# shicaiwei123/ICCV2025-GDL

Measured on AMD Instinct MI355X. Metric: audio-visual samples/sec, CREMA-D DGL train step (whole job), higher is better.
Workload: dtype bf16; 1 GPU; CREMA-D DGL (main_dgl.py, ConcatFusion_DGL) ResNet18 a+v, spec 1x257x188 + frames 3x3x224x224, alpha=4, SGD lr 2e-3 mom .9 wd 1e-4, clip 40; per_gpu_batch=64, global_batch=64, parallelism=dp1, buckets=none

## Files before the change

### iccv2025-gdl_amd/csrc/conv_wgrad.hip

```cpp
#include <stdlib.h>

#include "common.h"
#include "gather.h"
#include "prof.h"

#include <hip/hip_ext.h>

namespace gdl {

struct WgradArgs {
    const void* dy;
    const void* x;
    float* partial;
    const GatherEntry* table;
    int C, K, RS, M;
    int nsplit, chunk;
    int tiles_k, tiles_c;
    unsigned dy_bytes, x_bytes;
    int delta[9];
    int split;
    int delta_hi[9];
#ifdef GDL_TIMING
    unsigned long long* dbg;
#endif
};
#ifdef GDL_TIMING
extern unsigned long long* g_timing_buf;
#endif

constexpr int WG_BP = 64;

__device__ __forceinline__ uint2 lds_tr16(const unsigned char* p) {
    s16x4_t v = __builtin_amdgcn_ds_read_tr16_b64_v4i16((__attribute__((address_space(3))) s16x4_t*)(p));
    return __builtin_bit_cast(uint2, v);
}

__device__ __forceinline__ void wg_dma16(__amdgpu_buffer_rsrc_t rsrc, unsigned char* lds_base, int voffset) {
#if defined(__HIP_DEVICE_COMPILE__)
    __builtin_amdgcn_raw_ptr_buffer_load_lds(rsrc, (__attribute__((address_space(3))) void*)lds_base, 16, voffset, 0, 0, 0);
#else
    (void)rsrc;
    (void)lds_base;
    (void)voffset;
#endif
}
__device__ __forceinline__ uint2 lds_tr16_asm(unsigned addr) {
    uint2 v;
    asm volatile("ds_read_b64_tr_b16 %0, %1" : "=v"(v) : "v"(addr));
    return v;
}
__device__ __forceinline__ float lds_read_f32_asm(unsigned addr) {
    float v;
    asm volatile("ds_read_b32 %0, %1" : "=v"(v) : "v"(addr));
    return v;
}
__device__ __forceinline__ void wg_lds_wait() {
    asm volatile("s_waitcnt lgkmcnt(0)" ::: "memory");
    __builtin_amdgcn_sched_barrier(0);
}

template <int PITCH>
__device__ __forceinline__ int wg_swz(int row) {
    if (PITCH == 128) return ((row >> 1) & 1) | (((row >> 3) & 1) << 1);
    return (row & 3) | (((row >> 3) & 1) << 2);
}

template <typename T, int TK, int TC>
__global__ __launch_bounds__(256) void conv_wgrad_kernel(WgradArgs a) {
    extern __shared__ __attribute__((aligned(16))) unsigned char smem[];
    constexpr int PK = TK * (int)sizeof(T), PC = TC * (int)sizeof(T);
    constexpr int STAGE = WG_BP * (PK + PC);
    constexpr int CPR_K = PK / 16, CPR_C = PC / 16;
    constexpr int LK = WG_BP * CPR_K / 256, LC = WG_BP * CPR_C / 256;
    constexpr int WTK = TK / 2, WTC = TC / 2, FK = WTK / 16, FC = WTC / 16;

    const int tid = threadIdx.x, lane = tid & 63, wave = tid >> 6;
    const int wk = wave & 1, wc = wave >> 1;

    const int RS = a.RS;
    const int per_slice = RS * a.tiles_k * a.tiles_c;
    const int L = xcd_linear(a.nsplit * per_slice);
    if (L < 0) return;
    const int slice = L / per_slice;
    int rem = L - slice * per_slice;
    const int tap = rem % RS;
    rem /= RS;
    const int kt = rem % a.tiles_k, ct = rem / a.tiles_k;
    const int k0 = kt * TK, c0 = ct * TC;

    const int m_begin = slice * a.chunk;
    const int m_end = min(a.M, m_begin + a.chunk);
    const int nst = (m_end - m_begin + WG_BP - 1) / WG_BP;

    const __amdgpu_buffer_rsrc_t rdy = __builtin_amdgcn_make_buffer_rsrc((void*)a.dy, 0, a.dy_bytes, 0x00020000);
    const __amdgpu_buffer_rsrc_t rx = __builtin_amdgcn_make_buffer_rsrc((void*)a.x, 0, a.x_bytes, 0x00020000);
    const int esz = (int)sizeof(T);
    const int tap_delta = a.delta[tap] + c0 * esz;
    int dy_off[LK];
#pragma unroll
    for (int i = 0; i < LK; ++i) {
        const int idx = tid + 256 * i;
        const int row = idx / CPR_K, pc = idx % CPR_K;
        const int ch = (((pc >> 1) ^ wg_swz<PK>(row)) << 1) | (pc & 1);
        dy_off[i] = (m_begin + row) * (a.K * esz) + k0 * esz + ch * 16;
    }
    int x_ch[LC];
    bool x_hi[LC];
#pragma unroll
    for (int i = 0; i < LC; ++i) {
        const int idx = tid + 256 * i;
        const int row = idx / CPR_C, pc = idx % CPR_C;
        const int lc = (((pc >> 1) ^ wg_swz<PC>(row)) << 1) | (pc & 1);
        x_hi[i] = a.split && lc >= CPR_C / 2;
        x_ch[i] = (x_hi[i] ? lc - CPR_C / 2 : lc) * 16;
    }
    const int tap_delta_hi = a.delta_hi[tap];
    GatherEntry ent[LC];
#pragma unroll
    for (int i = 0; i < LC; ++i) {
        const int idx = tid + 256 * i;
        const int m = m_begin + idx / CPR_C;
        ent[i].off0 = 0;
        ent[i].mask = 0;
        if (m < m_end) ent[i] = a.table[m];
    }
    int ld_m = m_begin;
    const int wbase = (tid >> 6) * 64 * 16;

    auto load_stage = [&](int buf) {
        unsigned char* Ks = smem + buf * STAGE;
        unsigned char* Cs = Ks + WG_BP * PK;
#pragma unroll
        for (int i = 0; i < LK; ++i) {
            const int idx = tid + 256 * i;
            const int m = ld_m + idx / CPR_K;
            wg_dma16(rdy, Ks + 256 * 16 * i + wbase, m < m_end ? dy_off[i] : (int)0x80000000);
            dy_off[i] += WG_BP * a.K * esz;
        }
#pragma unroll
        for (int i = 0; i < LC; ++i) {
            const int v = ((ent[i].mask >> tap) & 1u) ? ent[i].off0 + (x_hi[i] ? tap_delta_hi : tap_delta) + x_ch[i]
                                                      : (int)0x80000000;
            wg_dma16(rx, Cs + 256 * 16 * i + wbase, v);
        }
        ld_m += WG_BP;
#pragma unroll
        for (int i = 0; i < LC; ++i) {
            const int idx = tid + 256 * i;
            const int m = ld_m + idx / CPR_C;
            GatherEntry e;
            e.off0 = 0;
            e.mask = 0;
            if (m < m_end) e = a.table[m];
            ent[i] = e;
        }
    };

    f32x4_t acc[FK][FC];
#pragma unroll
    for (int i = 0; i < FK; ++i)
#pragma unroll
        for (int jj = 0; jj < FC; ++jj) acc[i][jj] = f32x4_t{0.f, 0.f, 0.f, 0.f};

    const int g = lane >> 4, li = lane & 15;

    const unsigned smem_base = (unsigned)(uintptr_t)(const __attribute__((address_space(3))) unsigned char*)smem;
#ifdef GDL_TIMING
    unsigned long long t_entry = __builtin_amdgcn_s_memtime(), t_wait = 0, t_comp = 0, t_issue = 0, t_a, t_b;
#endif
    if (nst > 0) load_stage(0);
#ifdef GDL_TIMING
    unsigned long long t_first = __builtin_amdgcn_s_memtime();
#endif
    for (int st = 0; st < nst; ++st) {
        const int buf = st & 1;
#ifdef GDL_TIMING
        t_a = __builtin_amdgcn_s_memtime();
#endif
        asm volatile("s_waitcnt vmcnt(0)" ::: "memory");
        __builtin_amdgcn_s_barrier();
        asm volatile("" ::: "memory");
#ifdef GDL_TIMING
        t_b = __builtin_amdgcn_s_memtime();
        t_wait += t_b - t_a;
#endif
        if (st + 1 < nst) load_stage(buf ^ 1);
#ifdef GDL_TIMING
        t_a = __builtin_amdgcn_s_memtime();
        t_issue += t_a - t_b;
#endif
        const unsigned Ks = smem_base + buf * STAGE;
        const unsigned Cs = Ks + WG_BP * PK;
        if (sizeof(T) == 2) {
#pragma unroll
            for (int ks = 0; ks < WG_BP / 32; ++ks) {
                uint2 alo[FK], ahi[FK], blo[FC], bhi[FC];
#pragma unroll
                for (int h = 0; h < 2; ++h) {
                    const int row = ks * 32 + g * 8 + h * 4 + (li >> 2);
#pragma unroll
                    for (int i = 0; i < FK; ++i) {
                        const int chb = (wk * WTK + i * 16 + (li & 3) * 4) * 2;
                        const int addr = row * PK + ((((chb >> 5) ^ wg_swz<PK>(row)) << 5) | (chb & 31));
                        if (h == 0)
                            alo[i] = lds_tr16_asm(Ks + addr);
                        else
                            ahi[i] = lds_tr16_asm(Ks + addr);
                    }
#pragma unroll
                    for (int jj = 0; jj < FC; ++jj) {
                        const int chb = (wc * WTC + jj * 16 + (li & 3) * 4) * 2;
                        const int addr = row * PC + ((((chb >> 5) ^ wg_swz<PC>(row)) << 5) | (chb & 31));
                        if (h == 0)
                            blo[jj] = lds_tr16_asm(Cs + addr);
                        else
                            bhi[jj] = lds_tr16_asm(Cs + addr);
                    }
                }
                wg_lds_wait();
#pragma unroll
                for (int i = 0; i < FK; ++i) {
                    const uint4 fa = make_uint4(alo[i].x, alo[i].y, ahi[i].x, ahi[i].y);
#pragma unroll
                    for (int jj = 0; jj < FC; ++jj) {
                        const uint4 fb = make_uint4(blo[jj].x, blo[jj].y, bhi[jj].x, bhi[jj].y);
                        acc[i][jj] = __builtin_amdgcn_mfma_f32_16x16x32_bf16(__builtin_bit_cast(bf16x8_t, fa),
                                                                           __builtin_bit_cast(bf16x8_t, fb), acc[i][jj], 0,
                                                                           0, 0);
                    }
                }
            }
        } else {
#pragma unroll 4
            for (int ks = 0; ks < WG_BP / 4; ++ks) {
                const int row = ks * 4 + g;
                float fa[FK], fb[FC];
#pragma unroll
                for (int i = 0; i < FK; ++i) {
                    const int chb = (wk * WTK + i * 16 + li) * 4;
                    fa[i] = lds_read_f32_asm(Ks + row * PK + ((((chb >> 5) ^ wg_swz<PK>(row)) << 5) | (chb & 31)));
                }
#pragma unroll
                for (int jj = 0; jj < FC; ++jj) {
                    const int chb = (wc * WTC + jj * 16 + li) * 4;
                    fb[jj] = lds_read_f32_asm(Cs + row * PC + ((((chb >> 5) ^ wg_swz<PC>(row)) << 5) | (chb & 31)));
                }
                wg_lds_wait();
#pragma unroll
                for (int i = 0; i < FK; ++i)
#pragma unroll
                    for (int jj = 0; jj < FC; ++jj)
                        acc[i][jj] = __builtin_amdgcn_mfma_f32_16x16x4f32(fa[i], fb[jj], acc[i][jj], 0, 0, 0);
            }
        }
    }
#ifdef GDL_TIMING
    unsigned long long t_loop_end = __builtin_amdgcn_s_memtime();
    t_comp = (t_loop_end - t_first) - t_wait - t_issue;
#endif
    float* part = a.partial + (size_t)slice * a.K * RS * a.C;
#pragma unroll
    for (int i = 0; i < FK; ++i)
#pragma unroll
        for (int jj = 0; jj < FC; ++jj) {
            const int c = c0 + wc * WTC + jj * 16 + li;
#pragma unroll
            for (int e = 0; e < 4; ++e) {
                const int k = k0 + wk * WTK + i * 16 + g * 4 + e;
                part[((size_t)k * RS + tap) * a.C + c] = acc[i][jj][e];
            }
        }
#ifdef GDL_TIMING
    if (a.dbg && tid == 0) {
        unsigned long long* d = a.dbg + (size_t)blockIdx.x * 8;
        d[0] = t_entry;
        d[1] = t_first - t_entry;
        d[2] = t_wait;
        d[3] = t_issue;
        d[4] = t_comp;
        d[5] = __builtin_amdgcn_s_memtime() - t_loop_end;
        d[6] = nst;
    }
#endif
}

template <int LANES>
__global__ __launch_bounds__(256) void wgrad_reduce_kernel(const float* __restrict__ partial, float* __restrict__ out,
                                                           int nsplit, int K, int RS, int C, int Cout) {
    constexpr int OUTS = 256 / LANES;
    __shared__ float red[LANES][OUTS];
    const size_t total = (size_t)K * RS * C;
    const int o = threadIdx.x % OUTS, l = threadIdx.x / OUTS;
    const size_t i = blockIdx.x * (size_t)OUTS + o;
    float s = 0.f;
    if (i < total)
        for (int sp = l; sp < nsplit; sp += LANES) s += partial[(size_t)sp * total + i];
    if (LANES > 1) {
        red[l][o] = s;
        __syncthreads();
        if (l == 0) {
            s = red[0][o];
#pragma unroll
            for (int j = 1; j < LANES; ++j) s += red[j][o];
        }
    }
    if (l == 0 && i < total) {
        const int c = (int)(i % C);
        const size_t t = i / C;
        const int rs = (int)(t % RS);
        const int k = (int)(t / RS);
        if (c < Cout) out[((size_t)k * Cout + c) * RS + rs] = s;
    }
}

bool conv_wgrad9_enabled();
bool conv_wgrad9_ok(int dtype, int W, int C, int K, int R, int S, int stride, int pad);
size_t conv_wgrad9_ws_bytes(int M, int C, int K);
int conv_wgrad9(const void* dy, const void* x, float* dw, const void* table, int N, int H, int W, int C, int K, void* ws,
                size_t ws_bytes, hipStream_t st);

struct WgradPlan {
    int tk, tc, nsplit, chunk;
};

static WgradPlan plan_wgrad(int M, int C, int K, int RS, bool gemm = false) {
    WgradPlan p;
    p.tk = (K % 128 == 0) ? 128 : 64;
    p.tc = (C % 128 == 0) ? 128 : 64;
    const int tiles = (K / p.tk) * (C / p.tc) * RS;
    static int forced = -1;
    if (forced < 0) {
        const char* e = tune_env("GDL_WGRAD_BLOCKS");
        forced = e ? atoi(e) : 0;
    }
    static int forced_gemm = -1;
    if (forced_gemm < 0) {
        const char* e = tune_env("GDL_WGRAD_GEMM_BLOCKS");
        forced_gemm = e ? atoi(e) : 0;
    }
    const int target = (gemm && forced_gemm > 0) ? forced_gemm : forced > 0 ? forced : (gemm ? 416 : 128);
    int ns = (target + tiles - 1) / tiles;
    const int max_ns = (M + 2 * WG_BP - 1) / (2 * WG_BP);
    if (ns > max_ns) ns = max_ns;
    if (ns < 1) ns = 1;
    int chunk = (M + ns - 1) / ns;
    chunk = (chunk + WG_BP - 1) / WG_BP * WG_BP;
    p.nsplit = (M + chunk - 1) / chunk;
    p.chunk = chunk;
    return p;
}

size_t conv_wgrad_ws_bytes(int M, int C, int K, int RS) {
    const WgradPlan p = plan_wgrad(M, C, K, RS, RS == 1);
    size_t b = (size_t)p.nsplit * K * RS * C * sizeof(float);
    if (RS == 9 && conv_wgrad9_enabled()) {
        const size_t b9 = conv_wgrad9_ws_bytes(M, C, K);
        if (b9 > b) b = b9;
    }
    return b;
}

template <typename T, int TK, int TC>
static int launch_wg(WgradArgs& a, hipStream_t st) {
    constexpr int BYTES = 2 * WG_BP * (TK + TC) * (int)sizeof(T);
    auto kfn = conv_wgrad_kernel<T, TK, TC>;
    static DevOnce attr_set;
    if (!attr_set) {
        hipError_t e = hipFuncSetAttribute((const void*)kfn, hipFuncAttributeMaxDynamicSharedMemorySize, BYTES);
        if (e != hipSuccess) return check_hip(e, "hipFuncSetAttribute(conv_wgrad)");
        attr_set = true;
    }
    const int per_slice = a.RS * a.tiles_k * a.tiles_c;
    const int grid = xcd_grid(a.nsplit * per_slice);
    static char pname[96] = "";
    if (!pname[0]) snprintf(pname, sizeof(pname), "gdl::conv_wgrad_kernel<%s, %d, %d>", prof_tname<T>(), TK, TC);
    ProfScope prof(pname, PROF_MFMA, st, 2.0 * (double)a.M * a.K * a.C * a.RS, true,
                   (double)a.dy_bytes + (double)a.x_bytes + 4.0 * (double)a.K * a.C * a.RS);
    hipExtLaunchKernelGGL(kfn, dim3(grid), dim3(256), BYTES, st, prof.e0(), prof.e1(), 0, a);
    GDL_CHECK_LAUNCH("conv_wgrad_kernel");
    return GDL_OK;
}

int conv_wgrad(int dtype, const void* dy, const void* x, float* dw, const void* table, int N, int H, int W, int C, int K,
               int R, int S, int stride, int pad, int Cout, void* ws, size_t ws_bytes, hipStream_t st) {
    GDL_REQUIRE(dtype == GDL_BF16 || dtype == GDL_F32, "wgrad: bad dtype %d", dtype);
    GDL_REQUIRE(table, "wgrad: gather table is null (build it with gdl_conv_build_table)");
    GDL_REQUIRE(C % 64 == 0 && K % 64 == 0, "wgrad: C=%d K=%d must be multiples of 64", C, K);
    if (Cout == C && conv_wgrad9_ok(dtype, W, C, K, R, S, stride, pad))
        return conv_wgrad9(dy, x, dw, table, N, H, W, C, K, ws, ws_bytes, st);
    GatherGeom g;
    int rc = gather_geom(GATHER_FWD, dtype, N, H, W, C, K, R, S, stride, pad, &g);
    if (rc) return rc;
    const int esz = dtype == GDL_BF16 ? 2 : 4;
    WgradArgs a{};
#ifdef GDL_TIMING
    a.dbg = g_timing_buf;
#endif
    a.dy = dy;
    a.x = x;
    a.table = (const GatherEntry*)table;
    a.C = C;
    a.K = K;
    a.RS = R * S;
    a.M = g.rows;
    for (int t = 0; t < 9; ++t) a.delta[t] = g.delta[t];
    GDL_REQUIRE(a.M < (1 << 24), "wgrad: M exceeds 2^24");
    GDL_REQUIRE((size_t)a.M * K * esz < (1UL << 31), "wgrad: dy exceeds 2 GiB");
    a.dy_bytes = (unsigned)((size_t)a.M * K * esz);
    a.x_bytes = (unsigned)((size_t)N * H * W * C * esz);
    const WgradPlan p = plan_wgrad(a.M, C, K, R * S, R == 1 && S == 1 && stride == 1);
    a.nsplit = p.nsplit;
    a.chunk = p.chunk;
    a.tiles_k = K / p.tk;
    a.tiles_c = C / p.tc;
    const size_t need = (size_t)p.nsplit * K * R * S * C * sizeof(float);
    if (ws_bytes < need || !ws) {
        set_error("wgrad: workspace %zu < %zu bytes", ws_bytes, need);
        return GDL_ERR_WORKSPACE;
    }
    a.partial = (float*)ws;
    if (dtype == GDL_BF16) {
        if (p.tk == 128 && p.tc == 128)
            rc = launch_wg<bf16, 128, 128>(a, st);
        else if (p.tk == 128)
            rc = launch_wg<bf16, 128, 64>(a, st);
        else if (p.tc == 128)
            rc = launch_wg<bf16, 64, 128>(a, st);
        else
            rc = launch_wg<bf16, 64, 64>(a, st);
    } else {
        if (p.tk == 128 && p.tc == 128)
            rc = launch_wg<float, 128, 128>(a, st);
        else if (p.tk == 128)
            rc = launch_wg<float, 128, 64>(a, st);
        else if (p.tc == 128)
            rc = launch_wg<float, 64, 128>(a, st);
        else
            rc = launch_wg<float, 64, 64>(a, st);
    }
    if (rc) return rc;
    const size_t total = (size_t)K * R * S * C;
#ifdef GDL_EXPERIMENT
    if (experiment_mask2() & 1) return GDL_OK;
#endif
    ProfScope prof(p.nsplit >= 64 ? "gdl::wgrad_reduce_kernel<16>" : (p.nsplit > 8 ? "gdl::wgrad_reduce_kernel<4>" : "gdl::wgrad_reduce_kernel<1>"),
                   PROF_HBM, st, (double)total * 4.0 * (p.nsplit + 1));
    if (p.nsplit >= 64)
        hipLaunchKernelGGL(wgrad_reduce_kernel<16>, dim3((unsigned)((total + 15) / 16)), dim3(256), 0, st, a.partial, dw,
                           p.nsplit, K, R * S, C, Cout);
    else if (p.nsplit > 8)
        hipLaunchKernelGGL(wgrad_reduce_kernel<4>, dim3((unsigned)((total + 63) / 64)), dim3(256), 0, st, a.partial, dw,
                           p.nsplit, K, R * S, C, Cout);
    else
        hipLaunchKernelGGL(wgrad_reduce_kernel<1>, dim3((unsigned)((total + 255) / 256)), dim3(256), 0, st, a.partial, dw,
                           p.nsplit, K, R * S, C, Cout);
    GDL_CHECK_LAUNCH("wgrad_reduce_kernel");
    return GDL_OK;
}

__global__ __launch_bounds__(256) void stem_wgrad_reduce_kernel(const float* __restrict__ partial, float* __restrict__ out,
                                                                int nsplit, int Cin) {
    __shared__ float4 red[16][16];
    constexpr int TILE4 = 64 * 4 * 64 / 4;
    const int o = threadIdx.x & 15, l = threadIdx.x >> 4;
    const int idx4 = blockIdx.x * 16 + o;
    const float4* p = (const float4*)partial + idx4;
    float4 s = make_float4(0.f, 0.f, 0.f, 0.f);
    int sp = l;
    for (; sp + 48 < nsplit; sp += 64) {
        const float4 v0 = p[(size_t)sp * TILE4], v1 = p[(size_t)(sp + 16) * TILE4];
        const float4 v2 = p[(size_t)(sp + 32) * TILE4], v3 = p[(size_t)(sp + 48) * TILE4];
        s.x += v0.x, s.y += v0.y, s.z += v0.z, s.w += v0.w;
        s.x += v1.x, s.y += v1.y, s.z += v1.z, s.w += v1.w;
        s.x += v2.x, s.y += v2.y, s.z += v2.z, s.w += v2.w;
        s.x += v3.x, s.y += v3.y, s.z += v3.z, s.w += v3.w;
    }
    for (; sp < nsplit; sp += 16) {
        const float4 v0 = p[(size_t)sp * TILE4];
        s.x += v0.x, s.y += v0.y, s.z += v0.z, s.w += v0.w;
    }
    red[l][o] = s;
    __syncthreads();
    if (l != 0) return;
#pragma unroll
    for (int jj = 1; jj < 16; ++jj) {
        const float4 v = red[jj][o];
        s.x += v.x, s.y += v.y, s.z += v.z, s.w += v.w;
    }
    const int q = idx4 & 15, tap = (idx4 >> 4) & 3, k = idx4 >> 6;
    const int r = 2 * tap + (q >> 3), px = q & 7;
    if (r < 7 && px < 7) {
        const float v[4] = {s.x, s.y, s.z, s.w};
        for (int c = 0; c < Cin; ++c) out[((k * Cin + c) * 7 + r) * 7 + px] = v[c];
    }
}

struct StemRowsArgs {
    const void* dy;
    const void* xp;
    float* partial;
    int P, Q, Hp, Wp, nseg;
    int stages, chunk, nsplit;
    unsigned dy_bytes, x_bytes;
};
constexpr int SR_PITCH = 1088, SR_XBYTES = 9 * 1024, SR_STAGE = 8192 + SR_XBYTES;
template <int OFF>
__device__ __forceinline__ uint2 sr_tr(unsigned addr) {
    uint2 v;
    asm volatile("ds_read_b64_tr_b16 %0, %1 offset:%2" : "=v"(v) : "v"(addr), "n"(OFF));
    return v;
}
template <int N>
__device__ __forceinline__ void sr_wait() {
    __builtin_amdgcn_sched_barrier(0);
    asm volatile("s_waitcnt lgkmcnt(%0)" ::"n"(N) : "memory");
    __builtin_amdgcn_sched_barrier(0);
}
__global__ __launch_bounds__(256) void stem_wgrad_rows_kernel(StemRowsArgs a) {
    extern __shared__ __attribute__((aligned(16))) unsigned char smem[];
    const int tid = threadIdx.x, lane = tid & 63, wave = __builtin_amdgcn_readfirstlane(tid >> 6);
    const int g = lane >> 4, li = lane & 15;
    const int slice = blockIdx.x;
    const int s_begin = slice * a.chunk, s_end = min(a.stages, s_begin + a.chunk);
    const int nst = s_end - s_begin;
    const unsigned smem_base = (unsigned)(uintptr_t)(const __attribute__((address_space(3))) unsigned char*)smem;
    const __amdgpu_buffer_rsrc_t rdy = __builtin_amdgcn_make_buffer_rsrc((void*)a.dy, 0, a.dy_bytes, 0x00020000);
    const __amdgpu_buffer_rsrc_t rx = __builtin_amdgcn_make_buffer_rsrc((void*)a.xp, 0, a.x_bytes, 0x00020000);

    const int prow = lane >> 3, pch = lane & 7;
    int dy_rel[2];
#pragma unroll
    for (int i = 0; i < 2; ++i) {
        const int row = (wave + 4 * i) * 8 + prow;
        const int ch = (((pch >> 1) ^ wg_swz<128>(row)) << 1) | (pch & 1);
        dy_rel[i] = row * 128 + ch * 16;
    }
    int x_rel[3];
#pragma unroll
    for (int i = 0; i < 3; ++i) {
        const int p = wave + 4 * i, off = 1024 * p + 16 * lane;
        const int row = off / SR_PITCH, col = off % SR_PITCH;
        x_rel[i] = (p < 9 && row < 8 && col < 1072) ? row * a.Wp * 8 + col : -1;
    }
    int ld_s = s_begin;
    auto load_stage = [&](int buf) {
        unsigned char* Ks = smem + buf * SR_STAGE;
        unsigned char* Xs = Ks + 8192;
        const int sg = ld_s % a.nseg, R = ld_s / a.nseg;
        const int n = R / a.P, oh = R - n * a.P;
        const int ow0 = min(64 * sg, a.Q - 64), first = 64 * sg - ow0;
        const int dy_base = (R * a.Q + ow0) * 128;
        const int x_base = ((n * a.Hp + 2 * oh) * a.Wp + 2 * ow0) * 8;
#pragma unroll
        for (int i = 0; i < 2; ++i) {
            const int row = (wave + 4 * i) * 8 + prow;
            wg_dma16(rdy, Ks + (wave + 4 * i) * 1024, row >= first ? dy_base + dy_rel[i] : (int)0x80000000);
        }
#pragma unroll
        for (int i = 0; i < 3; ++i)
            if (wave + 4 * i < 9) wg_dma16(rx, Xs + (wave + 4 * i) * 1024, x_rel[i] >= 0 ? x_base + x_rel[i] : (int)0x80000000);
        ld_s += 1;
    };

    const int lrow = g * 8 + (li >> 2);
    unsigned aaddr[4][2], baddr[4][2];
#pragma unroll
    for (int h = 0; h < 2; ++h) {
        const int row = lrow + h * 4;
#pragma unroll
        for (int i = 0; i < 4; ++i) aaddr[i][h] = smem_base + row * 128 + ((i ^ wg_swz<128>(row)) << 5) + (li & 3) * 8;
#pragma unroll
        for (int t = 0; t < 4; ++t)
            baddr[t][h] = smem_base + 8192 + (2 * t + (wave >> 1)) * SR_PITCH + (2 * row + 4 * (wave & 1) + (li & 3)) * 8;
    }
    f32x4_t acc[4][4];
#pragma unroll
    for (int t = 0; t < 4; ++t)
#pragma unroll
        for (int i = 0; i < 4; ++i) acc[t][i] = f32x4_t{0.f, 0.f, 0.f, 0.f};

    if (nst > 0) load_stage(0);
    for (int st = 0; st < nst; ++st) {
        asm volatile("s_waitcnt vmcnt(0)" ::: "memory");
        __builtin_amdgcn_s_barrier();
        asm volatile("" ::: "memory");
        if (st + 1 < nst) load_stage((st + 1) & 1);
#pragma unroll
        for (int ks = 0; ks < 2; ++ks) {
            uint2 af[4][2], bf[4][2];
#pragma unroll
            for (int i = 0; i < 4; ++i)
#pragma unroll
                for (int h = 0; h < 2; ++h) af[i][h] = ks ? sr_tr<4096>(aaddr[i][h]) : sr_tr<0>(aaddr[i][h]);
#pragma unroll
            for (int t = 0; t < 4; ++t)
#pragma unroll
                for (int h = 0; h < 2; ++h) bf[t][h] = ks ? sr_tr<512>(baddr[t][h]) : sr_tr<0>(baddr[t][h]);
#pragma unroll
            for (int t = 0; t < 4; ++t) {
                if (t == 0)
                    sr_wait<6>();
                else if (t == 1)
                    sr_wait<4>();
                else if (t == 2)
                    sr_wait<2>();
                else
                    sr_wait<0>();
                const uint4 fb = make_uint4(bf[t][0].x, bf[t][0].y, bf[t][1].x, bf[t][1].y);
#pragma unroll
                for (int i = 0; i < 4; ++i) {
                    const uint4 fa = make_uint4(af[i][0].x, af[i][0].y, af[i][1].x, af[i][1].y);
                    acc[t][i] = __builtin_amdgcn_mfma_f32_16x16x32_bf16(__builtin_bit_cast(bf16x8_t, fa),
                                                                       __builtin_bit_cast(bf16x8_t, fb), acc[t][i], 0, 0, 0);
                }
            }
        }
        const int dlt = (st & 1) ? -SR_STAGE : SR_STAGE;
#pragma unroll
        for (int h = 0; h < 2; ++h) {
#pragma unroll
            for (int i = 0; i < 4; ++i) aaddr[i][h] += dlt;
#pragma unroll
            for (int t = 0; t < 4; ++t) baddr[t][h] += dlt;
        }
    }
    float* part = a.partial + (size_t)slice * (64 * 4 * 64);
#pragma unroll
    for (int t = 0; t < 4; ++t)
#pragma unroll
        for (int i = 0; i < 4; ++i)
#pragma unroll
            for (int e = 0; e < 4; ++e) part[((16 * i + g * 4 + e) * 4 + t) * 64 + 16 * wave + li] = acc[t][i][e];
}
struct StemFusedArgs {
    const void* y0;
    const void* dz;
    const uint8_t* idx;
    const float *scale, *shift, *mean, *rstd, *gamma, *coef;
    const void* xp;
    float* partial;
    int P, Q, PP, QQ, Hp, Wp, nseg;
    int stages, chunk, nsplit;
    unsigned x_bytes, y_bytes, dz_bytes;
#ifdef GDL_TIMING
    unsigned long long* dbg;
#endif
};
typedef unsigned int sr_u32x4_t __attribute__((ext_vector_type(4)));
__device__ __forceinline__ void sr_write16(unsigned addr, const uint4& v) {
    const sr_u32x4_t w = {v.x, v.y, v.z, v.w};
    asm volatile("ds_write_b128 %0, %1" ::"v"(addr), "v"(w) : "memory");
}
__global__ __launch_bounds__(256, 2) void stem_bwd_fused_kernel(StemFusedArgs a) {
    extern __shared__ __attribute__((aligned(16))) unsigned char smem[];
    const int tid = threadIdx.x, lane = tid & 63, wave = __builtin_amdgcn_readfirstlane(tid >> 6);
    const int g = lane >> 4, li = lane & 15;
    const int slice = blockIdx.x;
    const int s_begin = slice * a.chunk, s_end = min(a.stages, s_begin + a.chunk);
    const int nst = s_end - s_begin;
    const unsigned smem_base = (unsigned)(uintptr_t)(const __attribute__((address_space(3))) unsigned char*)smem;
    const __amdgpu_buffer_rsrc_t rx = __builtin_amdgcn_make_buffer_rsrc((void*)a.xp, 0, a.x_bytes, 0x00020000);

    const int vc = tid & 7;
    float sc[8], sf[8], A[8], Bc[8], D[8];
    {
        float mu[8], rs[8], gr[8], k1[8], k2[8];
#pragma unroll
        for (int q4 = 0; q4 < 2; ++q4) {
            auto ld = [&](const float* p, float* v) {
                const float4 t = *(const float4*)(p + vc * 8 + 4 * q4);
                v[4 * q4 + 0] = t.x, v[4 * q4 + 1] = t.y, v[4 * q4 + 2] = t.z, v[4 * q4 + 3] = t.w;
            };
            ld(a.scale, sc), ld(a.shift, sf), ld(a.mean, mu), ld(a.rstd, rs), ld(a.gamma, gr), ld(a.coef, k1), ld(a.coef + 64, k2);
        }
#pragma unroll
        for (int e = 0; e < 8; ++e) {
            A[e] = gr[e] * rs[e];
            Bc[e] = -A[e] * rs[e] * k2[e];
            D[e] = -A[e] * k1[e] - Bc[e] * mu[e];
        }
    }
    const int j2 = (tid >> 3) * 2;
    unsigned eoffs[2];
#pragma unroll
    for (int i = 0; i < 2; ++i) eoffs[i] = (j2 + i) * 128 + ((((vc >> 1) ^ wg_swz<128>(j2 + i)) << 5) | ((vc & 1) << 4));

    int x_rel[3];
#pragma unroll
    for (int i = 0; i < 3; ++i) {
        const int p = wave + 4 * i, off = 1024 * p + 16 * lane;
        const int row = off / SR_PITCH, col = off % SR_PITCH;
        x_rel[i] = (p < 9 && row < 8 && col < 1072) ? row * a.Wp * 8 + col : -1;
    }
    struct Coord {
        int sg, oh, n;
    };
    auto advance = [&](Coord& c) {
        if (++c.sg == a.nseg) {
            c.sg = 0;
            if (++c.oh == a.P) {
                c.oh = 0;
                ++c.n;
            }
        }
    };
    Coord cq;
    {
        const int R = s_begin / a.nseg;
        cq.sg = s_begin - R * a.nseg;
        cq.n = R / a.P;
        cq.oh = R - cq.n * a.P;
    }
    uint4 y_e, y_o, d_e[2], d_o[4];
    uint2 i_e[2], i_o[4];
    bool live_e = false, live_o = false;
    const uint4 z4 = make_uint4(0u, 0u, 0u, 0u);
    const __amdgpu_buffer_rsrc_t ry = __builtin_amdgcn_make_buffer_rsrc((void*)a.y0, 0, a.y_bytes, 0x00020000);
    const __amdgpu_buffer_rsrc_t rdz = __builtin_amdgcn_make_buffer_rsrc((void*)a.dz, 0, a.dz_bytes, 0x00020000);
    const __amdgpu_buffer_rsrc_t ridx = __builtin_amdgcn_make_buffer_rsrc((void*)a.idx, 0, a.dz_bytes >> 1, 0x00020000);
    auto bl16 = [](__amdgpu_buffer_rsrc_t r, int off) __attribute__((always_inline)) {
        const sr_u32x4_t v = __builtin_amdgcn_raw_buffer_load_b128(r, off, 0, 0);
        return make_uint4(v.x, v.y, v.z, v.w);
    };
    typedef unsigned int sr_u32x2_t __attribute__((ext_vector_type(2)));
    auto bl8 = [](__amdgpu_buffer_rsrc_t r, int off) __attribute__((always_inline)) {
        const sr_u32x2_t v = __builtin_amdgcn_raw_buffer_load_b64(r, off, 0, 0);
        return make_uint2(v.x, v.y);
    };
    constexpr int OOB = (int)0x80000000;
    auto request = [&](const Coord& c) {
        const int ow0 = min(64 * c.sg, a.Q - 64), first = 64 * c.sg - ow0;
        const int par = ow0 & 1;
        const int r_e = j2 + par, r_o = j2 + (par ^ 1);
        live_e = r_e >= first, live_o = r_o >= first;
        const int p = c.oh >> 1, hb = c.oh & 1;
        const int rowbase = (c.n * a.P + c.oh) * a.Q + ow0;
        const int q_e = (ow0 + r_e) >> 1, q_o = (ow0 + r_o) >> 1;
        const int w0 = (c.n * a.PP + p) * a.QQ;
        const bool row1 = hb && p + 1 < a.PP;
        const int w1 = row1 ? w0 + a.QQ : -1;
        const bool o1 = live_o && q_o + 1 < a.QQ;
        y_e = bl16(ry, live_e ? (rowbase + r_e) * 128 + vc * 16 : OOB);
        y_o = bl16(ry, live_o ? (rowbase + r_o) * 128 + vc * 16 : OOB);
        const int we = live_e ? (w0 + q_e) * 64 + vc * 8 : OOB, wo = live_o ? (w0 + q_o) * 64 + vc * 8 : OOB;
        const int wo1 = o1 ? (w0 + q_o + 1) * 64 + vc * 8 : OOB;
        d_e[0] = bl16(rdz, live_e ? (w0 + q_e) * 128 + vc * 16 : OOB), i_e[0] = bl8(ridx, we);
        d_o[0] = bl16(rdz, live_o ? (w0 + q_o) * 128 + vc * 16 : OOB), i_o[0] = bl8(ridx, wo);
        d_o[1] = bl16(rdz, o1 ? (w0 + q_o + 1) * 128 + vc * 16 : OOB), i_o[1] = bl8(ridx, wo1);
        const bool e2 = live_e && row1, o2 = live_o && row1, o3 = o1 && row1;
        d_e[1] = bl16(rdz, e2 ? (w1 + q_e) * 128 + vc * 16 : OOB), i_e[1] = bl8(ridx, e2 ? (w1 + q_e) * 64 + vc * 8 : OOB);
        d_o[2] = bl16(rdz, o2 ? (w1 + q_o) * 128 + vc * 16 : OOB), i_o[2] = bl8(ridx, o2 ? (w1 + q_o) * 64 + vc * 8 : OOB);
        d_o[3] = bl16(rdz, o3 ? (w1 + q_o + 1) * 128 + vc * 16 : OOB), i_o[3] = bl8(ridx, o3 ? (w1 + q_o + 1) * 64 + vc * 8 : OOB);
    };
    auto window = [&](float (&gsum)[8], const uint4& dq, const uint2& u, uint32_t code) __attribute__((always_inline)) {
        float d[8];
        unpack16<bf16>(dq, d);
#pragma unroll
        for (int c = 0; c < 4; ++c) {
            if (((u.x >> (8 * c)) & 0xff) == code) gsum[c] += d[c];
            if (((u.y >> (8 * c)) & 0xff) == code) gsum[4 + c] += d[4 + c];
        }
    };
    auto finish = [&](float (&gsum)[8], const uint4& yq, bool live, unsigned addr) __attribute__((always_inline)) {
        float yv[8];
        unpack16<bf16>(yq, yv);
#pragma unroll
        for (int c = 0; c < 8; ++c) {
            const float gg = (yv[c] * sc[c] + sf[c] > 0.f) ? gsum[c] : 0.f;
            gsum[c] = A[c] * gg + (Bc[c] * yv[c] + D[c]);
        }
        sr_write16(addr, live ? pack16<bf16>(gsum) : z4);
    };
    auto emit = [&](const Coord& c, int buf) {
        const int ow0 = min(64 * c.sg, a.Q - 64);
        const int par = ow0 & 1;
        const uint32_t hb = (uint32_t)(c.oh & 1);
        const unsigned base = smem_base + buf * SR_STAGE;
        float ge[8], go[8];
#pragma unroll
        for (int k = 0; k < 8; ++k) ge[k] = go[k] = 0.f;
        window(ge, d_e[0], i_e[0], (1 + hb) * 3 + 1);
        window(go, d_o[0], i_o[0], (1 + hb) * 3 + 2);
        window(go, d_o[1], i_o[1], (1 + hb) * 3);
        if (hb) {
            window(ge, d_e[1], i_e[1], 1);
            window(go, d_o[2], i_o[2], 2);
            window(go, d_o[3], i_o[3], 0);
        }
        finish(ge, y_e, live_e, base + eoffs[par]);
        finish(go, y_o, live_o, base + eoffs[par ^ 1]);
    };
    auto load_x = [&](const Coord& c, int buf) {
        unsigned char* Xs = smem + buf * SR_STAGE + 8192;
        const int ow0 = min(64 * c.sg, a.Q - 64);
        const int x_base = ((c.n * a.Hp + 2 * c.oh) * a.Wp + 2 * ow0) * 8;
#pragma unroll
        for (int i = 0; i < 3; ++i)
            if (wave + 4 * i < 9) wg_dma16(rx, Xs + (wave + 4 * i) * 1024, x_rel[i] >= 0 ? x_base + x_rel[i] : (int)0x80000000);
    };

    const int lrow = g * 8 + (li >> 2);
    unsigned aaddr[4][2], baddr[4][2];
#pragma unroll
    for (int h = 0; h < 2; ++h) {
        const int row = lrow + h * 4;
#pragma unroll
        for (int i = 0; i < 4; ++i) aaddr[i][h] = smem_base + row * 128 + ((i ^ wg_swz<128>(row)) << 5) + (li & 3) * 8;
#pragma unroll
        for (int t = 0; t < 4; ++t)
            baddr[t][h] = smem_base + 8192 + (2 * t + (wave >> 1)) * SR_PITCH + (2 * row + 4 * (wave & 1) + (li & 3)) * 8;
    }
    f32x4_t acc[4][4];
#pragma unroll
    for (int t = 0; t < 4; ++t)
#pragma unroll
        for (int i = 0; i < 4; ++i) acc[t][i] = f32x4_t{0.f, 0.f, 0.f, 0.f};

#ifdef GDL_TIMING
    unsigned long long t_entry = __builtin_amdgcn_s_memtime(), t_wait = 0, t_emit = 0, t_mul = 0, t_a, t_b;
#endif
    if (nst > 0) {
        request(cq);
        load_x(cq, 0);
        emit(cq, 0);
        if (nst > 1) {
            advance(cq);
            request(cq);
        }
    }
#ifdef GDL_TIMING
    const unsigned long long t_first = __builtin_amdgcn_s_memtime();
#endif
    for (int st = 0; st < nst; ++st) {
#ifdef GDL_TIMING
        t_a = __builtin_amdgcn_s_memtime();
#endif
        asm volatile("s_waitcnt vmcnt(0) lgkmcnt(0)" ::: "memory");
        __builtin_amdgcn_s_barrier();
        asm volatile("" ::: "memory");
#ifdef GDL_TIMING
        t_b = __builtin_amdgcn_s_memtime();
        t_wait += t_b - t_a;
#endif
        if (st + 1 < nst) {
            emit(cq, (st + 1) & 1);
            load_x(cq, (st + 1) & 1);
            if (st + 2 < nst) {
                advance(cq);
                request(cq);
            }
        }
#ifdef GDL_TIMING
        asm volatile("s_waitcnt lgkmcnt(0)" ::: "memory");
        t_a = __builtin_amdgcn_s_memtime();
        t_emit += t_a - t_b;
#endif
#pragma unroll
        for (int ks = 0; ks < 2; ++ks) {
            uint2 af[4][2], bf[4][2];
#pragma unroll
            for (int i = 0; i < 4; ++i)
#pragma unroll
                for (int h = 0; h < 2; ++h) af[i][h] = ks ? sr_tr<4096>(aaddr[i][h]) : sr_tr<0>(aaddr[i][h]);
#pragma unroll
            for (int t = 0; t < 4; ++t)
#pragma unroll
                for (int h = 0; h < 2; ++h) bf[t][h] = ks ? sr_tr<512>(baddr[t][h]) : sr_tr<0>(baddr[t][h]);
#pragma unroll
            for (int t = 0; t < 4; ++t) {
                if (t == 0)
                    sr_wait<6>();
                else if (t == 1)
                    sr_wait<4>();
                else if (t == 2)
                    sr_wait<2>();
                else
                    sr_wait<0>();
                const uint4 fb = make_uint4(bf[t][0].x, bf[t][0].y, bf[t][1].x, bf[t][1].y);
#pragma unroll
                for (int i = 0; i < 4; ++i) {
                    const uint4 fa = make_uint4(af[i][0].x, af[i][0].y, af[i][1].x, af[i][1].y);
                    acc[t][i] = __builtin_amdgcn_mfma_f32_16x16x32_bf16(__builtin_bit_cast(bf16x8_t, fa),
                                                                       __builtin_bit_cast(bf16x8_t, fb), acc[t][i], 0, 0, 0);
                }
            }
        }
#ifdef GDL_TIMING
        t_mul += __builtin_amdgcn_s_memtime() - t_a;
#endif
        const int dlt = (st & 1) ? -SR_STAGE : SR_STAGE;
#pragma unroll
        for (int h = 0; h < 2; ++h) {
#pragma unroll
            for (int i = 0; i < 4; ++i) aaddr[i][h] += dlt;
#pragma unroll
            for (int t = 0; t < 4; ++t) baddr[t][h] += dlt;
        }
    }
#ifdef GDL_TIMING
    if (a.dbg && lane == 0) {
        unsigned long long* d = a.dbg + ((size_t)blockIdx.x * 4 + wave) * 8;
        d[0] = t_entry, d[1] = t_first - t_entry, d[2] = t_wait, d[3] = t_emit, d[4] = t_mul;
        d[5] = __builtin_amdgcn_s_memtime() - t_first, d[6] = nst, d[7] = 0;
    }
#endif
    float* part = a.partial + (size_t)slice * (64 * 4 * 64);
#pragma unroll
    for (int t = 0; t < 4; ++t)
#pragma unroll
        for (int i = 0; i < 4; ++i)
#pragma unroll
            for (int e = 0; e < 4; ++e) part[((16 * i + g * 4 + e) * 4 + t) * 64 + 16 * wave + li] = acc[t][i][e];
}
struct StemRowsPlan {
    int nseg, stages, chunk, nsplit;
};
static bool stem_rows_ok(int dtype, int W) {
    static int v = -1;
    if (v < 0) {
        const char* e = tune_env("GDL_STEM_ROWS");
        v = e ? atoi(e) : 1;
    }
    return v != 0 && dtype == GDL_BF16 && (W - 1) / 2 + 1 >= 64;
}
static StemRowsPlan plan_stem_rows(int n_img, int H, int W) {
    const int P = (H - 1) / 2 + 1, Q = (W - 1) / 2 + 1;
    StemRowsPlan p;
    p.nseg = (Q + 63) / 64;
    p.stages = n_img * P * p.nseg;
    static int target = -1;
    if (target < 0) {
        const char* e = tune_env("GDL_STEM_ROWS_BLOCKS");
        target = e ? atoi(e) : 512;
    }
    int ns = target;
    if (ns > (p.stages + 3) / 4) ns = (p.stages + 3) / 4;
    if (ns < 1) ns = 1;
    p.chunk = (p.stages + ns - 1) / ns;
    p.nsplit = (p.stages + p.chunk - 1) / p.chunk;
    return p;
}

static WgradPlan plan_stem_wgrad(int M) { return plan_wgrad(M, 64, 64, 4); }
size_t conv_stem_wgrad_ws_bytes(int n_img, int H, int W) {
    const int M = n_img * ((H - 1) / 2 + 1) * ((W - 1) / 2 + 1);
    int ns = plan_stem_wgrad(M).nsplit;
    if ((W - 1) / 2 + 1 >= 64) ns = max(ns, plan_stem_rows(n_img, H, W).nsplit);
    return (size_t)ns * 64 * 4 * 64 * sizeof(float);
}
int conv_stem_wgrad(int dtype, const void* dy, const void* xp, float* dw, const void* table, int n_img, int H, int W, int Cin,
                    void* ws, size_t ws_bytes, hipStream_t st) {
    GDL_REQUIRE(dtype == GDL_BF16 || dtype == GDL_F32, "stem wgrad: bad dtype %d", dtype);
    GDL_REQUIRE(dy && xp && dw && table, "stem wgrad: null pointer");
    const int P = (H - 1) / 2 + 1, Q = (W - 1) / 2 + 1, Hp = H + 6, Wp = W + 8;
    const int esz = dtype == GDL_BF16 ? 2 : 4, pix = 4 * esz;
    if (stem_rows_ok(dtype, W)) {
        const StemRowsPlan p = plan_stem_rows(n_img, H, W);
        const size_t need = (size_t)p.nsplit * 64 * 4 * 64 * sizeof(float);
        if (ws_bytes < need || !ws) {
            set_error("stem wgrad: workspace %zu < %zu bytes", ws_bytes, need);
            return GDL_ERR_WORKSPACE;
        }
        GDL_REQUIRE((size_t)n_img * P * Q * 128 < (1UL << 31) && (size_t)n_img * Hp * Wp * 8 < (1UL << 31), "stem wgrad: tensor exceeds 2 GiB");
        StemRowsArgs r{};
        r.dy = dy;
        r.xp = xp;
        r.partial = (float*)ws;
        r.P = P, r.Q = Q, r.Hp = Hp, r.Wp = Wp, r.nseg = p.nseg;
        r.stages = p.stages, r.chunk = p.chunk, r.nsplit = p.nsplit;
        r.dy_bytes = (unsigned)((size_t)n_img * P * Q * 128);
        r.x_bytes = (unsigned)((size_t)n_img * Hp * Wp * 8);
        {
            ProfScope prof("gdl::stem_wgrad_rows_kernel", PROF_MFMA, st, 2.0 * (double)n_img * P * Q * 64 * 49 * Cin, true);
            hipExtLaunchKernelGGL(stem_wgrad_rows_kernel, dim3(p.nsplit), dim3(256), 2 * SR_STAGE, st, prof.e0(), prof.e1(), 0, r);
            GDL_CHECK_LAUNCH("stem_wgrad_rows_kernel");
        }
        ProfScope prof("gdl::stem_wgrad_reduce_kernel", PROF_HBM, st, (double)64 * Cin * 49 * 4.0 * (p.nsplit + 1));
        hipLaunchKernelGGL(stem_wgrad_reduce_kernel, dim3(64 * 4 * 64 / 4 / 16), dim3(256), 0, st, r.partial, dw, p.nsplit,
                           Cin);
        GDL_CHECK_LAUNCH("stem_wgrad_reduce_kernel");
        return GDL_OK;
    }
    WgradArgs a{};
#ifdef GDL_TIMING
    a.dbg = nullptr;
#endif
    a.dy = dy;
    a.x = xp;
    a.table = (const GatherEntry*)table;
    a.C = 64;
    a.K = 64;
    a.RS = 4;
    a.M = n_img * P * Q;
    a.split = 1;
    for (int t = 0; t < 4; ++t) {
        a.delta[t] = (2 * t) * Wp * pix;
        a.delta_hi[t] = 2 * t + 1 < 7 ? (2 * t + 1) * Wp * pix : 0x40000000;
    }
    GDL_REQUIRE(a.M < (1 << 24), "stem wgrad: M exceeds 2^24");
    GDL_REQUIRE((size_t)a.M * 64 * esz < (1UL << 31), "stem wgrad: dy exceeds 2 GiB");
    a.dy_bytes = (unsigned)((size_t)a.M * 64 * esz);
    a.x_bytes = (unsigned)((size_t)n_img * Hp * Wp * pix);
    const WgradPlan p = plan_stem_wgrad(a.M);
    a.nsplit = p.nsplit;
    a.chunk = p.chunk;
    a.tiles_k = 1;
    a.tiles_c = 1;
    const size_t need = (size_t)p.nsplit * 64 * 4 * 64 * sizeof(float);
    if (ws_bytes < need || !ws) {
        set_error("stem wgrad: workspace %zu < %zu bytes", ws_bytes, need);
        return GDL_ERR_WORKSPACE;
    }
    a.partial = (float*)ws;
    int rc = dtype == GDL_BF16 ? launch_wg<bf16, 64, 64>(a, st) : launch_wg<float, 64, 64>(a, st);
    if (rc) return rc;
    ProfScope prof("gdl::stem_wgrad_reduce_kernel", PROF_HBM, st, (double)64 * Cin * 49 * 4.0 * (p.nsplit + 1));
    hipLaunchKernelGGL(stem_wgrad_reduce_kernel, dim3(64 * 4 * 64 / 4 / 16), dim3(256), 0, st, a.partial, dw, p.nsplit,
                       Cin);
    GDL_CHECK_LAUNCH("stem_wgrad_reduce_kernel");
    return GDL_OK;
}

bool stem_bwd_fused_ok(int dtype, int W) {
    static int v = -1;
    if (v < 0) {
        const char* e = tune_env("GDL_STEM_FUSED");
        v = e ? atoi(e) : 1;
    }
    return v != 0 && stem_rows_ok(dtype, W);
}
int stem_bwd_fused(const void* dz, const uint8_t* idx, const void* y0, const float* scale, const float* shift, const float* mean,
                   const float* rstd, const float* gamma, const float* coef, const void* xp, float* dw, int n_img, int H, int W,
                   int Cin, void* ws, size_t ws_bytes, hipStream_t st) {
    GDL_REQUIRE(dz && idx && y0 && scale && shift && mean && rstd && gamma && coef && xp && dw, "stem_bwd_fused: null pointer");
    const int P = (H - 1) / 2 + 1, Q = (W - 1) / 2 + 1, Hp = H + 6, Wp = W + 8;
    GDL_REQUIRE(Q >= 64, "stem_bwd_fused: output rows of %d pixels (at least 64)", Q);
    const StemRowsPlan p = plan_stem_rows(n_img, H, W);
    const size_t need = (size_t)p.nsplit * 64 * 4 * 64 * sizeof(float);
    if (ws_bytes < need || !ws) {
        set_error("stem_bwd_fused: workspace %zu < %zu bytes", ws_bytes, need);
        return GDL_ERR_WORKSPACE;
    }
    GDL_REQUIRE((size_t)n_img * P * Q * 128 < (1UL << 31) && (size_t)n_img * Hp * Wp * 8 < (1UL << 31), "stem_bwd_fused: tensor exceeds 2 GiB");
    StemFusedArgs r{};
    r.y0 = y0, r.dz = dz, r.idx = idx;
    r.scale = scale, r.shift = shift, r.mean = mean, r.rstd = rstd, r.gamma = gamma, r.coef = coef;
    r.xp = xp;
    r.partial = (float*)ws;
    r.P = P, r.Q = Q, r.PP = (P - 1) / 2 + 1, r.QQ = (Q - 1) / 2 + 1, r.Hp = Hp, r.Wp = Wp, r.nseg = p.nseg;
    r.stages = p.stages, r.chunk = p.chunk, r.nsplit = p.nsplit;
    r.x_bytes = (unsigned)((size_t)n_img * Hp * Wp * 8);
    r.y_bytes = (unsigned)((size_t)n_img * P * Q * 128);
#ifdef GDL_TIMING
    r.dbg = g_timing_buf;
#endif
    r.dz_bytes = (unsigned)((size_t)n_img * r.PP * r.QQ * 128);
    {
        ProfScope prof("gdl::stem_bwd_fused_kernel", PROF_MFMA, st, 2.0 * (double)n_img * P * Q * 64 * 49 * Cin, true,
                       (double)n_img * P * Q * 128.0 + (double)n_img * r.PP * r.QQ * 192.0 + (double)n_img * Hp * Wp * 8.0);
        hipExtLaunchKernelGGL(stem_bwd_fused_kernel, dim3(p.nsplit), dim3(256), 2 * SR_STAGE, st, prof.e0(), prof.e1(), 0, r);
        GDL_CHECK_LAUNCH("stem_bwd_fused_kernel");
    }
    ProfScope prof("gdl::stem_wgrad_reduce_kernel", PROF_HBM, st, (double)64 * Cin * 49 * 4.0 * (p.nsplit + 1));
    hipLaunchKernelGGL(stem_wgrad_reduce_kernel, dim3(64 * 4 * 64 / 4 / 16), dim3(256), 0, st, r.partial, dw, p.nsplit, Cin);
    GDL_CHECK_LAUNCH("stem_wgrad_reduce_kernel");
    return GDL_OK;
}

}
```

Before: 13160 samples/s.

## Rotate epilogue rows per wave, skip dead rows, unroll stage loop by buffer parity

The fused stem wgrad kernel now gives each wave a rotating 16-row slice of the dy tile (by wave+oh), and skips loads and math for rows that fall before the segment start, writing zeros to LDS instead. The main loop is unrolled by double-buffer parity so LDS read offsets become compile-time immediates, which removes the per-stage address pointer updates. Window codes are kept in scalar registers to steer code generation. This changes the row-to-wave mapping and the LDS write layout, so it relies on the eoffs/rw*2048 layout matching the existing MFMA read addressing.

Result: no change. 13200 samples/s (median of 2 runs) (+0.3%).

```diff
diff --git a/iccv2025-gdl_amd/csrc/conv_wgrad.hip b/iccv2025-gdl_amd/csrc/conv_wgrad.hip
--- a/iccv2025-gdl_amd/csrc/conv_wgrad.hip
+++ b/iccv2025-gdl_amd/csrc/conv_wgrad.hip
@@ -1,4 +1,6 @@
 #include <stdlib.h>
+
+#include <type_traits>
 
 #include "common.h"
 #include "gather.h"
@@ -680,10 +682,12 @@
             D[e] = -A[e] * k1[e] - Bc[e] * mu[e];
         }
     }
-    const int j2 = (tid >> 3) * 2;
+    const int jl2 = (lane >> 3) * 2;
     unsigned eoffs[2];
 #pragma unroll
-    for (int i = 0; i < 2; ++i) eoffs[i] = (j2 + i) * 128 + ((((vc >> 1) ^ wg_swz<128>(j2 + i)) << 5) | ((vc & 1) << 4));
+    for (int i = 0; i < 2; ++i) eoffs[i] = (jl2 + i) * 128 + ((((vc >> 1) ^ wg_swz<128>(jl2 + i)) << 5) | ((vc & 1) << 4));
+    uint32_t code0 = 0, code1 = 1, code2 = 2;
+    asm volatile("" : "+s"(code0), "+s"(code1), "+s"(code2));
 
     int x_rel[3];
 #pragma unroll
@@ -730,7 +734,9 @@
     constexpr int OOB = (int)0x80000000;
     auto request = [&](const Coord& c) {
         const int ow0 = min(64 * c.sg, a.Q - 64), first = 64 * c.sg - ow0;
-        const int par = ow0 & 1;
+        const int rw = (wave + c.oh) & 3;
+        if (16 * rw + 16 <= first) return;
+        const int par = ow0 & 1, j2 = 16 * rw + jl2;
         const int r_e = j2 + par, r_o = j2 + (par ^ 1);
         live_e = r_e >= first, live_o = r_o >= first;
         const int p = c.oh >> 1, hb = c.oh & 1;
@@ -772,10 +778,15 @@
         sr_write16(addr, live ? pack16<bf16>(gsum) : z4);
     };
     auto emit = [&](const Coord& c, int buf) {
-        const int ow0 = min(64 * c.sg, a.Q - 64);
-        const int par = ow0 & 1;
+        const int ow0 = min(64 * c.sg, a.Q - 64), first = 64 * c.sg - ow0;
+        const int par = ow0 & 1, rw = (wave + c.oh) & 3;
         const uint32_t hb = (uint32_t)(c.oh & 1);
-        const unsigned base = smem_base + buf * SR_STAGE;
+        const unsigned base = smem_base + buf * SR_STAGE + rw * 2048;
+        if (16 * rw + 16 <= first) {
+            sr_write16(base + eoffs[0], z4);
+            sr_write16(base + eoffs[1], z4);
+            return;
+        }
         float ge[8], go[8];
 #pragma unroll
         for (int k = 0; k < 8; ++k) ge[k] = go[k] = 0.f;
@@ -783,9 +794,9 @@
         window(go, d_o[0], i_o[0], (1 + hb) * 3 + 2);
         window(go, d_o[1], i_o[1], (1 + hb) * 3);
         if (hb) {
-            window(ge, d_e[1], i_e[1], 1);
-            window(go, d_o[2], i_o[2], 2);
-            window(go, d_o[3], i_o[3], 0);
+            window(ge, d_e[1], i_e[1], code1);
+            window(go, d_o[2], i_o[2], code2);
+            window(go, d_o[3], i_o[3], code0);
         }
         finish(ge, y_e, live_e, base + eoffs[par]);
         finish(go, y_o, live_o, base + eoffs[par ^ 1]);
@@ -831,7 +842,8 @@
 #ifdef GDL_TIMING
     const unsigned long long t_first = __builtin_amdgcn_s_memtime();
 #endif
-    for (int st = 0; st < nst; ++st) {
+    auto stage = [&](auto BUF, int st) __attribute__((always_inline)) {
+        constexpr int RD = decltype(BUF)::value * SR_STAGE, NEXT = decltype(BUF)::value ^ 1;
 #ifdef GDL_TIMING
         t_a = __builtin_amdgcn_s_memtime();
 #endif
@@ -843,8 +855,8 @@
         t_wait += t_b - t_a;
 #endif
         if (st + 1 < nst) {
-            emit(cq, (st + 1) & 1);
-            load_x(cq, (st + 1) & 1);
+            emit(cq, NEXT);
+            load_x(cq, NEXT);
             if (st + 2 < nst) {
                 advance(cq);
                 request(cq);
@@ -861,11 +873,11 @@
 #pragma unroll
             for (int i = 0; i < 4; ++i)
 #pragma unroll
-                for (int h = 0; h < 2; ++h) af[i][h] = ks ? sr_tr<4096>(aaddr[i][h]) : sr_tr<0>(aaddr[i][h]);
+                for (int h = 0; h < 2; ++h) af[i][h] = ks ? sr_tr<RD + 4096>(aaddr[i][h]) : sr_tr<RD>(aaddr[i][h]);
 #pragma unroll
             for (int t = 0; t < 4; ++t)
 #pragma unroll
-                for (int h = 0; h < 2; ++h) bf[t][h] = ks ? sr_tr<512>(baddr[t][h]) : sr_tr<0>(baddr[t][h]);
+                for (int h = 0; h < 2; ++h) bf[t][h] = ks ? sr_tr<RD + 512>(baddr[t][h]) : sr_tr<RD>(baddr[t][h]);
 #pragma unroll
             for (int t = 0; t < 4; ++t) {
                 if (t == 0)
@@ -888,14 +900,10 @@
 #ifdef GDL_TIMING
         t_mul += __builtin_amdgcn_s_memtime() - t_a;
 #endif
-        const int dlt = (st & 1) ? -SR_STAGE : SR_STAGE;
-#pragma unroll
-        for (int h = 0; h < 2; ++h) {
-#pragma unroll
-            for (int i = 0; i < 4; ++i) aaddr[i][h] += dlt;
-#pragma unroll
-            for (int t = 0; t < 4; ++t) baddr[t][h] += dlt;
-        }
+    };
+    for (int st = 0; st < nst; st += 2) {
+        stage(std::integral_constant<int, 0>{}, st);
+        if (st + 1 < nst) stage(std::integral_constant<int, 1>{}, st + 1);
     }
 #ifdef GDL_TIMING
     if (a.dbg && lane == 0) {
```
